# king159/Pair-Net

Hardware: AMD Instinct MI355X
Metric: images/sec (whole node), 100-query 800x1333, 1/2/4/8 MI355X (higher is better)
Workload: dtype f32

## Files before the change

include/pairnet_hip.h:

```cpp
#ifndef PAIRNET_HIP_H_
#define PAIRNET_HIP_H_

#include <stdint.h>

#ifdef __cplusplus
extern "C" {
#endif

#define PN_ABI_VERSION 34
int pn_abi_version(void);

#define PN_GEMM_RELU       1
#define PN_GEMM_A_COLMAJOR 2
#define PN_GEMM_FORCE_TILE 4
#define PN_GEMM_FORCE_SKINNY 8
#define PN_GEMM_FORCE_TILE64 16
#define PN_GEMM_FORCE_TILE128x64 32
#define PN_GEMM_RELU_AFTER_RES 128
#define PN_GEMM_GELU 256
#define PN_GEMM_RESERVE_SHIFT 16
#define PN_GEMM_RESERVE(n) ((((n) / 8) & 0x3ff) << PN_GEMM_RESERVE_SHIFT)
#define PN_GEMM_KSPLIT_SHIFT 26
#define PN_GEMM_KSPLIT(n) (((n) & 31) << PN_GEMM_KSPLIT_SHIFT)

// ... 408 lines not shown
int pn_layernorm_rows_bwd_f32(const float* dy, int64_t lddy, const float* x, int64_t ldx,
                              const float* gamma, float* dx, int64_t lddx, float* gxhat,
                              int64_t ldg, int64_t rows, int C, float eps, void* stream);
int pn_gelu_f32(const float* x, float* y, int64_t n, void* stream);
int pn_gelu_bwd_f32(const float* dy, const float* x, float* dx, int64_t n, void* stream);
int pn_window_attention_bwd_f32(const float* qkv, int64_t ldqkv, const float* qkv_bias,
                                const float* bias_table, const float* dout, int64_t lddo,
                                const float* out, int64_t ldo, float* dqkv, int64_t lddqkv,
                                float* dtable_part, int B, int H, int W, int C, int heads, int ws,
                                int shift, float scale, void* stream);
int pn_patch_merge_ln_bwd_f32(const float* dy, const float* x, const float* gamma, float* dx,
                              float* part, int nblocks, int B, int H, int W, int C, float eps,
                              int accumulate, void* stream);
int pn_conv_weight_bwd_layout_f32(const float* in, float* out, int Co, int T, int Ci, void* stream);
int pn_dropout_f32(const float* x, const float* res , float* y, int64_t n, float p,
                   uint64_t seed, uint32_t subseq, uint32_t step, uint32_t site, void* stream);
int pn_dropout_keep_u8(uint8_t* keep, int64_t n, float p, uint64_t seed, uint32_t subseq,
                       uint32_t step, uint32_t site, void* stream);

int pn_grad_norm_clip_f32(const float* g, int64_t n, float pre, float max_norm, float* out,
                          double* scratch, void* stream);
int pn_adamw_f32(float* p, const float* g, float* m, float* v, int64_t n, const int64_t* seg_off,
                 const float* seg_lr, const float* seg_wd, int nseg, float lr, double beta1,
                 double beta2, float eps, float weight_decay, int step, const float* clip, float pre,
                 void* stream);
int pn_adamw_guarded_f32(float* p, const float* g, float* m, float* v, int64_t n,
                         const int64_t* seg_off, const float* seg_lr, const float* seg_wd, int nseg,
                         float lr, double beta1, double beta2, float eps, float weight_decay,
                         int step, const float* clip, float pre, const int32_t* guard, void* stream);

int64_t pn_s3_bytes(int rows, int K);
int pn_s3_split_f32(const float* X, int64_t ld, const float* add, int add_rows, void* S, int rows,
                    int K, void* stream);
int pn_s3_join_f32(const void* S, float* X, int64_t ld, int rows, int K, void* stream);
typedef struct pn_gemm_s3_desc {
  const void* A;  const void* A2;  int32_t a2_from_col;
  const void* W;  const float* bias;
  int32_t M, N, K;
  int32_t relu;
  float* C;       int64_t ldc;
  void* CS;
  void* CS_pos;   const float* pos;  int32_t pos_rows;
  const void* res_s3;  const float* gamma;  const float* beta;  float eps;
  int32_t flags;
  int32_t act;  const float* res;  int64_t ldres;
} pn_gemm_s3_desc;
#define PN_GEMM_S3_TILE96 1
#define PN_GEMM_S3_TILE192 2
int pn_gemm_s3_f32(const pn_gemm_s3_desc* d, void* stream);
typedef struct pn_gemm_s3_ffn_desc {
  const void* X;  const void* W1;  const float* b1;
  const void* W2; const float* b2;
  int32_t M, N, K, F;
  int32_t act;
  float* C;       int64_t ldc;
  void* CS;
  void* CS_pos;   const float* pos;  int32_t pos_rows;
  const void* res_s3;  const float* gamma;  const float* beta;  float eps;
} pn_gemm_s3_ffn_desc;
int pn_gemm_s3_ffn_f32(const pn_gemm_s3_ffn_desc* d, void* stream);

int pn_uniform_f32(float* out, int64_t n, int nsites, uint32_t site_stride, uint64_t seed,
                   uint32_t rank, uint32_t step, uint32_t site, void* stream);
int pn_seg_targets(const int64_t* table, const int32_t* row_ind, const int32_t* col_ind,
                   const int32_t* lsa_status, int nlsa, const int64_t* gt_labels, int64_t gt_len,
                   int64_t out_len, int L, int B, int Q, int C, int64_t Mtot, int64_t* labels,
                   int64_t* matched, int32_t* mcount, int32_t* status, void* stream);
int pn_uncertain_points_f32(const float* maps, int64_t nmaps, const int64_t* matched, int64_t M,
                            int B, int Q, int h, int w, const float* cand, const float* tail, int S,
                            int k, int Np, uint32_t* keys, float* pts, void* stream);
int pn_point_sample_rows_f32(const void* maps, int maps_are_u8, int64_t nmaps, const int64_t* idx,
                             const float* pts, float* out, int64_t M, int h, int w, int Np,
                             void* stream);
int pn_mask_point_loss_f32(const float* x, const float* t, const int64_t* matched, int64_t M, int Np,
                           int L, int Ml, float w_mask, float w_dice, float dice_eps,
                           float num_total_masks, float* sums, float* out , float* coef,
                           void* stream);
int64_t pn_point_scatter_scratch_ints(int64_t M, int Np, int h, int w);
int pn_point_scatter_grad_f32(const float* coef, const float* pts, float* grad, int32_t* scratch,
                              int64_t M, int Np, int h, int w, void* stream);
int pn_ce_avg_f32(const float* logits, const int64_t* target, const float* class_weight, float* out,
                  int L, int rows, int C, float loss_weight, void* stream);
int pn_ce_avg_grad_f32(const float* logits, const int64_t* target, const float* class_weight,
                       float* grad, int L, int rows, int C, float loss_weight, void* stream);

int pn_rel_id_cost_f32(const float* rel, const float* sub, const float* obj, const int64_t* gt_rels,
                       int64_t rel_len, const int64_t* matched, int64_t Mtot, const int64_t* tab,
                       float* cost, int64_t cost_len, int B, int R, int Q, int C1, float w_s,
                       float w_o, float w_r, void* stream);
int pn_rel_targets(const int64_t* tab, const int32_t* row_ind, const int32_t* col_ind,
                   int64_t out_len, const int32_t* lsa_status, const int64_t* gt_rels,
                   int64_t rel_len, const int64_t* matched, int64_t Mtot, int B, int R, int Q, int C1,
                   int64_t* r_labels, int32_t* pos, int32_t* status, void* stream);
// ... 62 lines not shown
```

pair-net_amd/csrc/gemm_s3.hip:

```cpp
#include "common.h"
#include "s3_common.h"

__device__ __forceinline__ void s3_glds16(const void* g, void* l) {
  __builtin_amdgcn_global_load_lds((const __attribute__((address_space(1))) void*)g,
                                   (__attribute__((address_space(3))) void*)l, 16, 0, 0);
}

__device__ __forceinline__ int64_t pos8_offset(int row, int col, int N) {
  return ((((int64_t)(row >> 5) * (N >> 4) + (col >> 4)) * 2 + ((col >> 3) & 1)) * 32 + (row & 31)) * 8;
}

__global__ __launch_bounds__(256) void k_s3_split(const float* __restrict__ X, int64_t ld,
                                                  const float* __restrict__ add, int add_rows,
                                                  uint4* __restrict__ S, int R, int K) {
  const int KB = K >> 4;
  const int lane = threadIdx.x & 63;
  const int64_t piece = (int64_t)blockIdx.x * 4 + (threadIdx.x >> 6);
  const int64_t npieces = (int64_t)((R + 31) >> 5) * KB;
  if (piece >= npieces) return;
  const int rb = (int)(piece / KB), kb = (int)(piece - (int64_t)rb * KB);
  const int r = rb * 32 + (lane & 31), k = kb * 16 + (lane >> 5) * 8;
  float v[8];
  if (r < R) {
    const float4 a = ld4(X + (int64_t)r * ld + k), b = ld4(X + (int64_t)r * ld + k + 4);
    v[0] = a.x; v[1] = a.y; v[2] = a.z; v[3] = a.w; v[4] = b.x; v[5] = b.y; v[6] = b.z; v[7] = b.w;
    if (add) {
      const float* p = add + (int64_t)(r % add_rows) * K + k;
      const float4 c = ld4(p), d = ld4(p + 4);
      v[0] += c.x; v[1] += c.y; v[2] += c.z; v[3] += c.w; v[4] += d.x; v[5] += d.y; v[6] += d.z; v[7] += d.w;
    }
  } else {
#pragma unroll
    for (int i = 0; i < 8; ++i) v[i] = 0.f;
  }
  s3_frag p0, p1, p2;
  s3_split8(v, p0, p1, p2);
  uint4* o = S + piece * 192 + lane;
  o[0] = p0.u; o[64] = p1.u; o[128] = p2.u;
}

__global__ __launch_bounds__(256) void k_s3_join(const uint4* __restrict__ S, float* __restrict__ X,
                                                 int64_t ld, int R, int K) {
  const int KB = K >> 4;
  const int lane = threadIdx.x & 63;
  const int64_t piece = (int64_t)blockIdx.x * 4 + (threadIdx.x >> 6);
  const int64_t npieces = (int64_t)((R + 31) >> 5) * KB;
  if (piece >= npieces) return;
  const int rb = (int)(piece / KB), kb = (int)(piece - (int64_t)rb * KB);
  const int r = rb * 32 + (lane & 31), k = kb * 16 + (lane >> 5) * 8;
  if (r >= R) return;
  const uint4* in = S + piece * 192 + lane;
  s3_frag p0, p1, p2;
  p0.u = in[0]; p1.u = in[64]; p2.u = in[128];
  float v[8];
  s3_join8(p0, p1, p2, v);
  st4(X + (int64_t)r * ld + k, make_float4(v[0], v[1], v[2], v[3]));
  st4(X + (int64_t)r * ld + k + 4, make_float4(v[4], v[5], v[6], v[7]));
}

struct s3_args {
  const uint4* A; const uint4* A2; int a2_from_tile;
  const uint4* W; const float* bias;
  float* C; int64_t ldc; uint4* CS; uint4* CSP;
  const uint4* RES; const float* gamma; const float* beta; const float* pos; int pos_rows; float eps;
  int M, N, K, relu;
  const float* res; int64_t ldres;
  int nout;
};

__device__ __forceinline__ void s3_block_epilogue(const f32x16& acc, const s3_args& p, int rb, int n0,
// ... 648 lines not shown
        read(u & 1, as);
        if (u < 7) issueW1(c, u + 1);
        else issueW2(c, 0);
        if (u + 2 < 8) issueA(u + 2, as2, 1);
        __builtin_amdgcn_s_setprio(0);
        bar();
        mma(acc1);
        drain_bar();
        as = as == 2 ? 0 : as + 1;
      }
      make_pieces(c);
      bar();
#pragma unroll 1
      for (int s = 0; s < 8; ++s) {
        const int as2 = as == 0 ? 2 : as - 1;
        const bool more = c + 1 < NC;
        __builtin_amdgcn_s_setprio(1);
        read(s & 1, as);
        if (s < 7) issueW2(c, s + 1);
        else if (more) issueW1(c + 1, 0);
        if (s >= 6 && more) issueA(s - 6, as2, 1);
        __builtin_amdgcn_s_setprio(0);
        bar();
        mma(acc2);
        if (wave == s + 2) write_pieces(as2);
        if (more || s < 7) drain_bar();
        as = as == 2 ? 0 : as + 1;
      }
    }
  }
  s3_ln_epilogue(acc2, p, smem, rb0, wave * 32, wave, lane);
}

__global__ __launch_bounds__(256) void k_gemm_s3_narrow(const s3_args p, const int col0) {
  const int lane = threadIdx.x & 63;
  const int KB = p.K >> 4, RB = (p.M + 31) >> 5, ncb = (p.N - col0) >> 5;
  const int unit = blockIdx.x * 4 + (threadIdx.x >> 6);
  if (unit >= RB * ncb) return;
  const int rb = unit / ncb, cb = (col0 >> 5) + unit - rb * ncb;
  const uint4* ga = ((p.A2 && (cb >> 3) >= p.a2_from_tile) ? p.A2 : p.A) + (int64_t)rb * KB * 192 + lane;
  const uint4* gw = p.W + (int64_t)cb * KB * 192 + lane;
  f32x16 acc;
#pragma unroll
  for (int r = 0; r < 16; ++r) acc[r] = 0.f;
  constexpr int PA[6] = {2, 1, 0, 1, 0, 0}, PB[6] = {0, 1, 2, 0, 1, 0};
  constexpr int D = 4;
  s3_frag a[D][3], b[D][3];
  auto load = [&](int kb, int slot) {
#pragma unroll
    for (int q = 0; q < 3; ++q) { a[slot][q].u = ga[kb * 192 + q * 64]; b[slot][q].u = gw[kb * 192 + q * 64]; }
  };
#pragma unroll
  for (int d = 0; d < D; ++d)
    if (d < KB) load(d, d);
  for (int kb = 0; kb < KB; kb += D) {
#pragma unroll
    for (int d = 0; d < D; ++d) {
      if (kb + d >= KB) break;
#pragma unroll
      for (int q = 0; q < 6; ++q)
        acc = __builtin_amdgcn_mfma_f32_32x32x16_bf16(b[d][PB[q]].v, a[d][PA[q]].v, acc, 0, 0, 0);
      if (kb + d + D < KB) load(kb + d + D, d);
    }
  }
  s3_block_epilogue(acc, p, rb, cb * 32, lane);
}

extern "C" int64_t pn_s3_bytes(int rows, int K) {
  return (int64_t)((rows + 31) / 32) * (K / 16) * 3072;
}

extern "C" int pn_s3_split_f32(const float* X, int64_t ld, const float* add, int add_rows, void* S,
                               int rows, int K, void* stream) {
  if (!X || !S || rows <= 0 || K <= 0 || K % 16 || ld % 4 || (add && add_rows <= 0)) return PN_BAD_ARG;
  const int64_t np = (int64_t)((rows + 31) / 32) * (K / 16);
  k_s3_split<<<dim3((unsigned)((np + 3) / 4)), dim3(256), 0, (hipStream_t)stream>>>(
      X, ld, add, add ? add_rows : 1, (uint4*)S, rows, K);
  return PN_LAUNCH_CHECK();
}

extern "C" int pn_s3_join_f32(const void* S, float* X, int64_t ld, int rows, int K, void* stream) {
  if (!X || !S || rows <= 0 || K <= 0 || K % 16 || ld % 4) return PN_BAD_ARG;
  const int64_t np = (int64_t)((rows + 31) / 32) * (K / 16);
  k_s3_join<<<dim3((unsigned)((np + 3) / 4)), dim3(256), 0, (hipStream_t)stream>>>(
      (const uint4*)S, X, ld, rows, K);
  return PN_LAUNCH_CHECK();
}

extern "C" int pn_gemm_s3_ffn_f32(const pn_gemm_s3_ffn_desc* d, void* stream) {
  if (!d || !d->X || !d->W1 || !d->W2 || d->M <= 0) return PN_BAD_ARG;
  if (d->K != 256 || d->N != 256 || d->F <= 0 || d->F % 256) return PN_BAD_ARG;
  if (d->act != 1) return PN_BAD_ARG;
  if (!d->gamma || !d->beta) return PN_BAD_ARG;
  if (!d->C && !d->CS && !d->CS_pos) return PN_BAD_ARG;
  if (d->C && (d->ldc % 4 || d->ldc < d->N)) return PN_BAD_ARG;
  if (d->CS_pos && (!d->pos || d->pos_rows <= 0)) return PN_BAD_ARG;
  s3_args a;
  a.A = (const uint4*)d->X; a.A2 = nullptr; a.a2_from_tile = 0;
  a.W = (const uint4*)d->W2; a.bias = d->b2;
  a.C = d->C; a.ldc = d->ldc; a.CS = (uint4*)d->CS; a.CSP = (uint4*)d->CS_pos;
  a.RES = (const uint4*)d->res_s3; a.gamma = d->gamma; a.beta = d->beta; a.pos = d->pos;
  a.pos_rows = d->pos_rows; a.eps = d->eps;
  a.M = d->M; a.N = d->N; a.K = d->F; a.relu = 0; a.nout = d->N;
  a.res = nullptr; a.ldres = 0;
  const int RB = (d->M + 31) / 32, mt = (RB + 2) / 3;
  k_gemm_s3_ffn<<<dim3(mt), dim3(512), 0, (hipStream_t)stream>>>(a, (const uint4*)d->W1, d->b1);
  return PN_LAUNCH_CHECK();
}

extern "C" int pn_gemm_s3_f32(const pn_gemm_s3_desc* d, void* stream) {
  if (!d || !d->A || !d->W || d->M <= 0 || d->N <= 0 || d->K <= 0) return PN_BAD_ARG;
  if (d->K % 32 || d->N % 32) return PN_BAD_ARG;
  if (!d->C && !d->CS && !d->CS_pos) return PN_BAD_ARG;
  if (d->C && (d->ldc % 4 || d->ldc < d->N)) return PN_BAD_ARG;
  if (d->A2 && (d->a2_from_col <= 0 || d->a2_from_col % 256)) return PN_BAD_ARG;
  if (d->CS_pos && (!d->pos || d->pos_rows <= 0)) return PN_BAD_ARG;
  const bool ln = d->gamma != nullptr;
  if (ln && (d->N != 256 || !d->beta || d->relu)) return PN_BAD_ARG;
  if (!ln && d->res_s3) return PN_BAD_ARG;
  if (d->res && (ln || d->ldres % 4 || d->ldres < d->N)) return PN_BAD_ARG;
  if (d->act < 0 || d->act > 3 || (ln && d->act)) return PN_BAD_ARG;
  s3_args a;
  a.A = (const uint4*)d->A; a.A2 = (const uint4*)d->A2; a.a2_from_tile = d->A2 ? d->a2_from_col / 256 : 0;
  a.W = (const uint4*)d->W; a.bias = d->bias;
  a.C = d->C; a.ldc = d->ldc; a.CS = (uint4*)d->CS; a.CSP = (uint4*)d->CS_pos;
  a.RES = (const uint4*)d->res_s3; a.gamma = d->gamma; a.beta = d->beta; a.pos = d->pos;
  a.pos_rows = d->pos_rows; a.eps = d->eps;
  a.M = d->M; a.N = d->N; a.K = d->K; a.relu = d->act ? d->act : d->relu; a.nout = d->N;
  a.res = d->res; a.ldres = d->ldres;
  const int rem = d->N % 256;
  const bool narrow = !ln && !d->CS_pos && d->N > 256 && rem > 0 && rem <= 64;
  const int RB = (d->M + 31) / 32, mt = (RB + 2) / 3;
  bool wide = !ln && !d->CS_pos && (d->N - (narrow ? rem : 0)) >= 512 && !(d->flags & PN_GEMM_S3_TILE96);
  if (wide && !(d->flags & PN_GEMM_S3_TILE192)) {
    static int cus = 0;
    if (!cus) {
      int dev = 0;
      if (hipGetDevice(&dev) != hipSuccess ||
          hipDeviceGetAttribute(&cus, hipDeviceAttributeMultiprocessorCount, dev) != hipSuccess || cus <= 0)
// ... 29 lines not shown
```

pair-net_amd/head.py:

```python
import math
from collections import OrderedDict

import torch

from . import hip
from . import plans
from .plans import Arena, PlanCache, measure_bytes
from .config import ConfigDict

INSTANCE_OFFSET = 1000


def _decoder_param_shapes(prefix, num_layers, ffn_dim, out):
    for i in range(num_layers):
        p = "%s.layers.%d." % (prefix, i)
        for a in (0, 1):
            out[p + "attentions.%d.attn.in_proj_weight" % a] = (768, 256)
            out[p + "attentions.%d.attn.in_proj_bias" % a] = (768,)
            out[p + "attentions.%d.attn.out_proj.weight" % a] = (256, 256)
            out[p + "attentions.%d.attn.out_proj.bias" % a] = (256,)
        out[p + "ffns.0.layers.0.0.weight"] = (ffn_dim, 256)
        out[p + "ffns.0.layers.0.0.bias"] = (ffn_dim,)
        out[p + "ffns.0.layers.1.weight"] = (256, ffn_dim)
        out[p + "ffns.0.layers.1.bias"] = (256,)
# ... 70 lines not shown
        self.num_enc_layers = pixel_decoder.encoder.num_layers
        self.enc_ffn = pixel_decoder.encoder.transformerlayers.ffn_cfgs.feedforward_channels
        self.gn_groups = pixel_decoder.norm_cfg.num_groups
        self.num_dec_layers = transformer_decoder.num_layers
        self.dec_ffn = transformer_decoder.transformerlayers.ffn_cfgs.feedforward_channels
        self.num_rel_layers = relation_decoder.num_layers
        self.rel_ffn = relation_decoder.transformerlayers.ffn_cfgs.feedforward_channels
        self.rel_ffn_drop = float(relation_decoder.transformerlayers.ffn_cfgs.get("ffn_drop", 0.0))
        self.other_drop_rates = _drop_rates(dict(pixel_decoder=pixel_decoder,
                                                 transformer_decoder=transformer_decoder,
                                                 relation_decoder=relation_decoder))
        self.other_drop_rates.pop("relation_decoder.transformerlayers.ffn_cfgs.ffn_drop", None)
        self.test_cfg, self.train_cfg = test_cfg, train_cfg
        assert len(self.in_channels) == 4 and num_transformer_feat_level == 3
        assert num_obj_query <= 256 and num_rel_query <= 128
        self._params = OrderedDict(
            (k, torch.zeros(s)) for k, s in self.param_shapes().items())
        self.device = None
        self.w = None
        self._plans = PlanCache()
        self._arenas, self._post_arenas, self._consts, self._pe = {}, {}, {}, OrderedDict()
        self._dummies = {}
        self._post = OrderedDict()
        self._pan_jobs = []
        self.graph_after = 1
        self.exact_mask_order = True
        self.conv_algo = "winograd4"
        self.use_graphs = False
        self.grid_reserve = 0
        self.fuse_ppn_front = True
        self.fuse_mask_pack = True
        self.gather_mask_stencil = True
        self.fuse_encoder_ffn = 1
        self.fuse_lateral_upadd = False
        self.enc_fused_ln = ("proj", "ffn")
        self.group_input_convs = False
        self.gemm_arithmetic = "bf16x3"
        self.msda_s3_out = False
        self.fused_pair_masks = True
        self.init_weights()

    def param_shapes(self):
        s = OrderedDict()
        Q, R = self.num_obj_query, self.num_rel_query
        _decoder_param_shapes("relation_decoder", self.num_rel_layers, self.rel_ffn, s)
        s["rel_query_embed.weight"] = (R, 256)
        s["rel_query_embed2.weight"] = (2 * R, 256)
        s["rel_query_embed3.weight"] = (2 * R, 256)
        s["rel_query_feat.weight"] = (R, 256)
        for i, (ci, co) in enumerate(((1, 64), (64, 64), (64, 1))):
            s["update_importance.conv_layers.%d.0.weight" % i] = (co, ci, 7, 7)
            s["update_importance.conv_layers.%d.0.bias" % i] = (co,)
        pd = "pixel_decoder."
        for i in range(3):
            cin = self.in_channels[3 - i]
            s[pd + "input_convs.%d.conv.weight" % i] = (256, cin, 1, 1)
            s[pd + "input_convs.%d.conv.bias" % i] = (256,)
            s[pd + "input_convs.%d.gn.weight" % i] = (256,)
            s[pd + "input_convs.%d.gn.bias" % i] = (256,)
        for i in range(self.num_enc_layers):
            p = pd + "encoder.layers.%d." % i
            for name, n in (("sampling_offsets", 192), ("attention_weights", 96),
                            ("value_proj", 256), ("output_proj", 256)):
                s[p + "attentions.0.%s.weight" % name] = (n, 256)
                s[p + "attentions.0.%s.bias" % name] = (n,)
            s[p + "ffns.0.layers.0.0.weight"] = (self.enc_ffn, 256)
# ... 464 lines not shown
        for i in range(self.num_enc_layers):
            p = pd + "encoder.layers.%d." % i
            a = p + "attentions.0."
            hip.gemm(X2, w[a + "voa.weight"], pl.VOA, M=B * SN, N=544, K=256, lda=256, ldw=256,
                     ldc=544, bias=w[a + "voa.bias"], aadd=pl.enc_pos, ldaadd=256, aadd_rows=SN,
                     aadd_from_col=256)
            hip.msda(pl.VOA, 544, pl.VOA.view(-1)[256:], 544, pl.S, B, pl.shapes)
            if "proj" in self.enc_fused_ln:
                hip.linear_res_ln(pl.S.view(-1, 256), w[a + "output_proj.weight"],
                                  w[a + "output_proj.bias"], X2, w[p + "norms.0.weight"],
                                  w[p + "norms.0.bias"], X12)
            else:
                hip.linear(pl.S.view(-1, 256), w[a + "output_proj.weight"],
                           w[a + "output_proj.bias"], Y2, res=X2)
                hip.layernorm(Y2, w[p + "norms.0.weight"], w[p + "norms.0.bias"], X12)
            hip.linear(X12, w[p + "ffns.0.layers.0.0.weight"], w[p + "ffns.0.layers.0.0.bias"],
                       pl.H, relu=True)
            if "ffn" in self.enc_fused_ln:
                hip.linear_res_ln(pl.H, w[p + "ffns.0.layers.1.weight"],
                                  w[p + "ffns.0.layers.1.bias"], X12, w[p + "norms.1.weight"],
                                  w[p + "norms.1.bias"], X2)
            else:
                hip.linear(pl.H, w[p + "ffns.0.layers.1.weight"], w[p + "ffns.0.layers.1.bias"],
                           Y2, res=X12)
                hip.layernorm(Y2, w[p + "norms.1.weight"], w[p + "norms.1.bias"], X2)

    def _encoder_s3(self, pl):
        w, B, SN = self.w, pl.B, pl.SN
        pd = "pixel_decoder."
        M, F = B * SN, self.enc_ffn
        X2 = pl.X.view(-1, 256)
        pos8 = (pl.enc_pos8, SN)
        fuse_ffn = bool(getattr(self, "fuse_encoder_ffn", 0)) and F % 256 == 0
        hip.s3_split(X2, pl.XS)
        hip.s3_split(X2, pl.XPS, add=pl.enc_pos)
        for i in range(self.num_enc_layers):
            p = pd + "encoder.layers.%d." % i
            a = p + "attentions.0."
            last = i + 1 == self.num_enc_layers
            hip.gemm_s3(pl.XS, w[a + "voa.weight.s3"], M, 544, 256, bias=w[a + "voa.bias"],
                        out=pl.VOA.view(-1, 544), a2=pl.XPS, a2_from_col=256)
            if self.msda_s3_out:
                hip.msda(pl.VOA, 544, pl.VOA.view(-1)[256:], 544, pl.SS, B, pl.shapes, s3_out=True)
            else:
                hip.msda(pl.VOA, 544, pl.VOA.view(-1)[256:], 544, pl.S, B, pl.shapes)
                hip.s3_split(pl.S.view(-1, 256), pl.SS)
            hip.gemm_s3(pl.SS, w[a + "output_proj.weight.s3"], M, 256, 256,
                        bias=w[a + "output_proj.bias"], out_s3=pl.X1S, res_s3=pl.XS,
                        gamma=w[p + "norms.0.weight"], beta=w[p + "norms.0.bias"])
            tail = dict(res_s3=pl.X1S, gamma=w[p + "norms.1.weight"], beta=w[p + "norms.1.bias"],
                        out=X2 if last else None, out_s3=None if last else pl.XS,
                        out_s3_pos=None if last else pl.XPS, pos=pos8)
            if fuse_ffn:
                hip.gemm_s3_ffn(pl.X1S, w[p + "ffns.0.layers.0.0.weight.s3"],
                                w[p + "ffns.0.layers.1.weight.s3"], M, 256, 256, F,
                                b1=w[p + "ffns.0.layers.0.0.bias"],
                                b2=w[p + "ffns.0.layers.1.bias"], **tail)
                continue
            hip.gemm_s3(pl.X1S, w[p + "ffns.0.layers.0.0.weight.s3"], M, F, 256,
                        bias=w[p + "ffns.0.layers.0.0.bias"], relu=True, out_s3=pl.HS)
            hip.gemm_s3(pl.HS, w[p + "ffns.0.layers.1.weight.s3"], M, 256, F,
                        bias=w[p + "ffns.0.layers.1.bias"], **tail)

    def _mlp3(self, prefix, src, dst, pl):
        w = self.w
        hip.linear(src, w[prefix + ".0.weight"], w[prefix + ".0.bias"], pl.m1, relu=True)
        hip.linear(pl.m1, w[prefix + ".2.weight"], w[prefix + ".2.bias"], pl.m2, relu=True)
        hip.linear(pl.m2, w[prefix + ".4.weight"], w[prefix + ".4.bias"], dst)

    def _mask_logits(self, me, pl, out):
        Q = self.num_obj_query
        hip.gemm(me, pl.MF, out, M=Q, N=pl.HW2, K=256, lda=256, ldw=256, ldc=pl.HW2,
                 batch=pl.B, sA=Q * 256, sW=pl.HW2 * 256, sC=Q * pl.HW2)

    def _head_embed(self, q, pl, with_cls, full_mask, cls_out=None, mp_out=None, normed=False):
        w, B, Q = self.w, pl.B, self.num_obj_query
        cls_out = pl.cls if cls_out is None else cls_out
        mp_out = pl.MP if mp_out is None else mp_out
        if not normed:
            hip.layernorm(q, w["transformer_decoder.post_norm.weight"],
                          w["transformer_decoder.post_norm.bias"], pl.qn)
        if with_cls:
# ... 185 lines not shown
        hip.gather_rows(pl.MP, pl.obj_pos, pl.obj_seg, B, Q, R, pl.HW2)

    def _outputs(self, pl):
        B, Q, R = pl.B, self.num_obj_query, self.num_rel_query
        H2, W2 = pl.hw2
        return (dict(sub=pl.sub_cls, obj=pl.obj_cls, cls=pl.cls, rel=pl.rel, importance=pl.imp),
                dict(mask=pl.MP.view(B, Q, H2, W2), sub_seg=pl.sub_seg.view(B, R, H2, W2),
                     obj_seg=pl.obj_seg.view(B, R, H2, W2)))

    def _check_feats(self, feats, img_metas):
        pv = getattr(self, "_packed_version", None)
        if self.w is not None and pv is not None and pv != self._weights_version():
            self._drop_weight_state()
        B = len(img_metas)
        assert len(feats) == 4 and all(f.shape[0] == B for f in feats)
        nchw = all(f.is_contiguous() for f in feats)
        nhwc = not nchw and all(f.is_contiguous(memory_format=torch.channels_last) for f in feats)
        for f, c in zip(feats, self.in_channels):
            if not f.is_cuda or f.dtype != torch.float32 or f.shape[1] != c or not (nchw or nhwc):
                raise RuntimeError("feats must be fp32 [B,C,H,W] device tensors with channels %s, "
                                   "all contiguous or all in channels_last memory format"
                                   % self.in_channels)
        if self.device is None:
            self.to(feats[0].device)
        shapes = [tuple(feats[3 - l].shape[-2:]) for l in range(3)]
        self._feats_nhwc = nhwc
        return B, shapes, tuple(feats[0].shape[-2:])

    def _run_stage(self, which, pl, feats=None):
        cfg = (self.exact_mask_order, self.conv_algo, self.fuse_ppn_front, self.grid_reserve,
               tuple(self.enc_fused_ln), self.group_input_convs,
               getattr(self, "fuse_mask_pack", True), self.gemm_arithmetic, self.msda_s3_out,
               self._fused_pair_masks(), bool(getattr(self, "fuse_encoder_ffn", 0)),
               getattr(self, "gather_mask_stencil", True), getattr(self, "fuse_lateral_upadd", False))
        if pl.graph_cfg != cfg:
            pl.graph_a = pl.graph_b = None
            pl.graphs_a = OrderedDict()
            pl.graph_c = PlanCache(self.POST_VIEWS)
            pl.graph_cfg = cfg
        cur = torch.cuda.current_stream(self.device)
        pl.streams[cur.cuda_stream] = cur
        try:
            self._run_stage_on(which, pl, feats, cur)
        finally:
            plans.note_use(cur)

    def _run_stage_on(self, which, pl, feats, cur):
        if which == "a":
            if not pl.pe_waited:
                if pl.pe_ready.query():
                    pl.pe_waited = True
                else:
                    cur.wait_event(pl.pe_ready)
            ptrs = tuple(f.data_ptr() for f in feats)
            ent = pl.graphs_a.get(ptrs)
            if ent is None:
                if len(pl.graphs_a) >= self.STAGE_A_GRAPHS:
                    for k, e in pl.graphs_a.items():
                        if e["graph"] is None:
                            del pl.graphs_a[k]
                            break
                    else:
                        if plans.quiet(cur):
                            torch.cuda.current_stream(self.device).synchronize()
                            pl.graphs_a.popitem(last=False)
                if len(pl.graphs_a) < self.STAGE_A_GRAPHS:
# ... 331 lines not shown
```

pair-net_amd/hip.py:

```python
import contextlib
import ctypes as C
import os
import threading

import torch

from .build import LIB_PATH

LIB_PATH = os.environ.get("PAIRNET_LIB") or LIB_PATH

_i32, _i64, _f32, _vp = C.c_int32, C.c_int64, C.c_float, C.c_void_p

GEMM_RELU, GEMM_A_COLMAJOR, GEMM_FORCE_TILE, GEMM_FORCE_SKINNY = 1, 2, 4, 8
GEMM_GELU = 256
GEMM_FORCE_TILE64, GEMM_FORCE_TILE128x64 = 16, 32
GEMM_RELU_AFTER_RES = 128
GEMM_GROUP_MAX = 18


class GemmDesc(C.Structure):
    _fields_ = [("A", _vp), ("lda", _i64), ("strideA", _i64),
                ("Aadd", _vp), ("ldaadd", _i64), ("aadd_rows", _i32),
                ("aadd_from_col", _i32),
                ("W", _vp), ("ldw", _i64), ("strideW", _i64),
                ("bias", _vp),
                ("Res", _vp), ("ldres", _i64), ("strideRes", _i64),
                ("C", _vp), ("ldc", _i64), ("strideC", _i64),
                ("M", _i32), ("N", _i32), ("K", _i32), ("batch", _i32),
                ("flags", _i32),
                ("splitk_scratch", _vp), ("splitk_scratch_floats", _i64)]


class GemmS3Desc(C.Structure):
    _fields_ = [("A", _vp), ("A2", _vp), ("a2_from_col", _i32),
                ("W", _vp), ("bias", _vp),
                ("M", _i32), ("N", _i32), ("K", _i32), ("relu", _i32),
                ("C", _vp), ("ldc", _i64),
                ("CS", _vp),
                ("CS_pos", _vp), ("pos", _vp), ("pos_rows", _i32),
                ("res_s3", _vp), ("gamma", _vp), ("beta", _vp), ("eps", _f32), ("flags", _i32),
                ("act", _i32), ("res", _vp), ("ldres", _i64)]


class GemmS3FfnDesc(C.Structure):
    _fields_ = [("X", _vp), ("W1", _vp), ("b1", _vp), ("W2", _vp), ("b2", _vp),
                ("M", _i32), ("N", _i32), ("K", _i32), ("F", _i32), ("act", _i32),
                ("C", _vp), ("ldc", _i64),
                ("CS", _vp),
                ("CS_pos", _vp), ("pos", _vp), ("pos_rows", _i32),
                ("res_s3", _vp), ("gamma", _vp), ("beta", _vp), ("eps", _f32)]


_SIGS = {
    "pn_abi_version": (C.c_int, []),
    "pn_s3_bytes": (_i64, [_i32, _i32]),
    "pn_s3_split_f32": (C.c_int, [_vp, _i64, _vp, _i32, _vp, _i32, _i32, _vp]),
    "pn_s3_join_f32": (C.c_int, [_vp, _vp, _i64, _i32, _i32, _vp]),
    "pn_gemm_s3_f32": (C.c_int, [C.POINTER(GemmS3Desc), _vp]),
    "pn_gemm_s3_ffn_f32": (C.c_int, [C.POINTER(GemmS3FfnDesc), _vp]),
    "pn_gemm_f32": (C.c_int, [C.POINTER(GemmDesc), _vp]),
    "pn_gemm_variant": (C.c_int, [C.POINTER(GemmDesc)]),
    "pn_gemm_grid_size": (C.c_int, [C.POINTER(GemmDesc)]),
    "pn_gemm_wgs_per_cu": (C.c_int, []),
    "pn_gemm_group_f32": (C.c_int, [C.POINTER(GemmDesc), C.c_int, _vp]),
    "pn_conv2d_nhwc_f32": (C.c_int, [_vp, _vp, _vp, _vp] + [_i32] * 10 + [_vp]),
    "pn_conv2d_nhwc_ex_f32": (C.c_int, [_vp] * 5 + [_i32] * 10 + [_vp, _i64, _vp]),
    "pn_bottleneck_proj_f32": (C.c_int, [_vp] * 8 + [_i32] * 8 + [_vp, _i64, _vp]),
    "pn_stem7x7s2_f32": (C.c_int, [_vp, _vp, _vp, _vp, _i32, _i32, _i32, _i32, _vp]),
    "pn_maxpool3x3s2_nhwc_f32": (C.c_int, [_vp, _vp, _i32, _i32, _i32, _i32, _vp]),
    "pn_winograd_f23_input_f32": (C.c_int, [_vp, _vp, _i32, _i32, _i32, _i32, _vp]),
    "pn_winograd_f23_output_f32": (C.c_int, [_vp, _vp, _vp, _i32, _i32, _i32, _i32, _i32, _vp]),
    "pn_winograd_f43_input_f32": (C.c_int, [_vp, _vp, _i32, _i32, _i32, _i32, _vp]),
    "pn_winograd_f43_output_f32": (C.c_int, [_vp, _vp, _vp, _i32, _i32, _i32, _i32, _i32, _vp]),
    "pn_layernorm_f32": (C.c_int, [_vp, _vp, _vp, _vp, _i64, _i32, _f32, _vp]),
    "pn_layernorm_rows_s3_f32": (C.c_int, [_vp, _i64, _vp, _vp, _vp, _i64, _i32, _f32, _vp]),
    "pn_layernorm_rows_f32": (C.c_int, [_vp, _i64, _vp, _vp, _vp, _i64, _i64, _i32, _f32, _vp]),
    "pn_patch_merge_ln_f32": (C.c_int, [_vp, _vp, _vp, _vp, _i32, _i32, _i32, _i32, _f32, _vp]),
    "pn_patch_im2col4_f32": (C.c_int, [_vp, _vp, _i32, _i32, _i32, _vp]),
    "pn_window_attention_f32": (C.c_int, [_vp, _i64, _vp, _vp, _vp, _i64] + [_i32] * 7 +
                                [_f32, _vp]),
    "pn_window_attention_s3_f32": (C.c_int, [_vp, _i64, _vp, _vp, _vp] + [_i32] * 7 + [_f32, _vp]),
    "pn_groupnorm_nblk": (C.c_int, [_i64]),
    "pn_groupnorm_nhwc_f32": (C.c_int, [_vp, _vp, _vp, _vp, _vp, _i32, _i64, _i32,
                                        _i32, _f32, _i32, _i64, _i64, _vp]),
    "pn_groupnorm_upadd_nhwc_f32": (C.c_int, [_vp] * 6 + [_i32] * 7 + [_f32, _i64, _i64, _i64, _vp]),
    "pn_l2normalize_f32": (C.c_int, [_vp, _vp, _i64, _i32, _f32, _vp]),
    "pn_ffn_scratch_floats": (_i64, [_i32, _i32]),
    "pn_ffn_ln_f32": (C.c_int, [_vp] * 9 + [_i32, _i32, _i32, _f32, _vp]),
    "pn_ffn_ln2_f32": (C.c_int, [_vp] * 12 + [_i32, _i32, _i32, _f32, _vp]),
    "pn_msda_f32": (C.c_int, [_vp, _i64, _vp, _i64, _vp, _i32, _i32, C.POINTER(_i32),
                              C.POINTER(_i32), _vp]),
    "pn_msda_ex_f32": (C.c_int, [_vp, _i64, _vp, _i64, _vp, _i32, _i32, C.POINTER(_i32),
# ... 519 lines not shown
def layernorm(x, gamma, beta, out, eps=1e-5):
    rows = x.numel() // 256
    _check(lib().pn_layernorm_f32(_ptr(x), _ptr(gamma), _ptr(beta), _ptr(out), rows, 256,
                                  eps, _stream()), "pn_layernorm_f32")


def linear_res_ln(x, weight, bias, res, gamma, beta, out, eps=1e-5):
    M, ldx = _rowmajor(x)
    N, ldw = _rowmajor(weight)
    Mr, ldr = _rowmajor(res)
    Mo, ldo = _rowmajor(out)
    K = x.shape[1]
    assert Mr == M and Mo == M and N == 256 and weight.shape[1] == K
    nbytes = 4.0 * (M * K + N * K + 2 * M * N)
    _check(_launch("k_gemm_rowln", 2.0 * M * N * K, nbytes,
                   lambda: lib().pn_linear_res_ln_f32(_ptr(x), ldx, _ptr(weight), ldw, _ptr(bias),
                                                      _ptr(res), ldr, _ptr(gamma), _ptr(beta),
                                                      _ptr(out), ldo, M, N, K, eps, _stream()),
                   meta=(M, N, K, 1, False)), "pn_linear_res_ln_f32")


def s3_floats(rows, K):
    return ((rows + 31) // 32) * (K // 16) * 768


def pos8(pos):
    rows, cols = pos.shape
    rb = (rows + 31) // 32
    p = pos.new_zeros(rb * 32, cols)
    p[:rows] = pos
    return p.view(rb, 32, cols // 16, 2, 8).permute(0, 2, 3, 1, 4).contiguous()


def s3_split(x, out, add=None):
    rows, ld = _rowmajor(x)
    K = x.shape[1]
    assert out.numel() * out.element_size() >= s3_floats(rows, K) * 4
    ar = 0
    if add is not None:
        ar, lda = _rowmajor(add)
        assert lda == K and add.shape[1] == K
    _check(_launch("k_s3_split", 0.0, 10.0 * rows * K,
                   lambda: lib().pn_s3_split_f32(_ptr(x), ld, _ptr(add), ar, _ptr(out), rows, K,
                                                 _stream())), "pn_s3_split_f32")


def s3_join(s3, out):
    rows, ld = _rowmajor(out)
    _check(_launch("k_s3_join", 0.0, 10.0 * rows * out.shape[1],
                   lambda: lib().pn_s3_join_f32(_ptr(s3), _ptr(out), ld, rows, out.shape[1],
                                                _stream())), "pn_s3_join_f32")


def gemm_s3(a, w, M, N, K, *, bias=None, relu=False, out=None, out_s3=None, out_s3_pos=None,
            pos=None, a2=None, a2_from_col=0, res_s3=None, gamma=None, beta=None, eps=1e-5,
            tile96=False, tile192=False, gelu=False, res=None, relu_after=False):
    d = GemmS3Desc()
    d.A, d.A2, d.a2_from_col = _ptr(a), _ptr(a2), a2_from_col
    d.W, d.bias = _ptr(w), _ptr(bias)
    d.M, d.N, d.K, d.relu = M, N, K, int(relu)
    if out is not None:
        Mo, ldc = _rowmajor(out)
        assert Mo == M and out.shape[1] >= N
        d.C, d.ldc = _ptr(out), ldc
    d.CS, d.CS_pos = _ptr(out_s3), _ptr(out_s3_pos)
    if out_s3_pos is not None:
        pos, pr = pos
        assert pos.numel() == (pr + 31) // 32 * 32 * N
        d.pos, d.pos_rows = _ptr(pos), pr
    d.res_s3, d.gamma, d.beta, d.eps = _ptr(res_s3), _ptr(gamma), _ptr(beta), eps
    d.flags = (1 if tile96 else 0) | (2 if tile192 else 0)
    d.act = 3 if relu_after else 2 if gelu else 0
    if res is not None:
        Mr, ldr = _rowmajor(res)
        assert Mr == M and res.shape[1] >= N
        d.res, d.ldres = _ptr(res), ldr
    nbytes = 6.0 * (M * K + N * K) + (4.0 * M * N if out is not None else 0.0) + \
        6.0 * M * N * ((out_s3 is not None) + (out_s3_pos is not None) + (res_s3 is not None))
    name = "k_gemm_s3<ln>" if gamma is not None else "k_gemm_s3"
    _check(_launch(name, 2.0 * M * N * K, nbytes, lambda: lib().pn_gemm_s3_f32(C.byref(d), _stream()),
                   meta=(M, N, K, 1, False)), "pn_gemm_s3_f32")


def gemm_s3_ffn(x, w1, w2, M, N, K, F, *, b1=None, b2=None, res_s3=None, gamma=None, beta=None,
                eps=1e-5, out=None, out_s3=None, out_s3_pos=None, pos=None, gelu=False):
    d = GemmS3FfnDesc()
    d.X, d.W1, d.b1, d.W2, d.b2 = _ptr(x), _ptr(w1), _ptr(b1), _ptr(w2), _ptr(b2)
    d.M, d.N, d.K, d.F, d.act = M, N, K, F, 2 if gelu else 1
    if out is not None:
        Mo, ldc = _rowmajor(out)
        assert Mo == M and out.shape[1] >= N
        d.C, d.ldc = _ptr(out), ldc
    d.CS, d.CS_pos = _ptr(out_s3), _ptr(out_s3_pos)
    if out_s3_pos is not None:
        pos, pr = pos
        assert pos.numel() == (pr + 31) // 32 * 32 * N
        d.pos, d.pos_rows = _ptr(pos), pr
    d.res_s3, d.gamma, d.beta, d.eps = _ptr(res_s3), _ptr(gamma), _ptr(beta), eps
    nbytes = 6.0 * (M * K + 2 * F * K) + (4.0 * M * N if out is not None else 0.0) + \
        6.0 * M * N * ((out_s3 is not None) + (out_s3_pos is not None) + (res_s3 is not None))
    _check(_launch("k_gemm_s3_ffn", 2.0 * M * F * (K + N), nbytes,
                   lambda: lib().pn_gemm_s3_ffn_f32(C.byref(d), _stream()),
                   meta=(M, N, F, 1, False)), "pn_gemm_s3_ffn_f32")


def layernorm_rows(x, gamma, beta, out, eps=1e-5):
    rows, ldx = _rowmajor(x)
    ro, ldo = _rowmajor(out)
    assert ro == rows and out.shape[1] == x.shape[1]
    _check(_launch("k_ln_rows", 0.0, 8.0 * rows * x.shape[1],
                   lambda: lib().pn_layernorm_rows_f32(_ptr(x), ldx, _ptr(gamma), _ptr(beta),
                                                       _ptr(out), ldo, rows, x.shape[1], eps,
                                                       _stream())), "pn_layernorm_rows_f32")


def layernorm_rows_s3(x, gamma, beta, out_s3, eps=1e-5):
    rows, ldx = _rowmajor(x)
    Cc = x.shape[1]
    assert out_s3.numel() >= s3_floats(rows, Cc)
    _check(_launch("k_ln_rows<s3>", 0.0, 10.0 * rows * Cc,
                   lambda: lib().pn_layernorm_rows_s3_f32(_ptr(x), ldx, _ptr(gamma), _ptr(beta),
                                                          _ptr(out_s3), rows, Cc, eps, _stream())),
           "pn_layernorm_rows_s3_f32")


def patch_merge_ln(x, gamma, beta, out, B, H, W, C, eps=1e-5):
    _check(_launch("k_ln_rows<merge>", 0.0, 8.0 * B * H * W * C,
                   lambda: lib().pn_patch_merge_ln_f32(_ptr(x), _ptr(gamma), _ptr(beta), _ptr(out),
                                                       B, H, W, C, eps, _stream())),
           "pn_patch_merge_ln_f32")


def patch_im2col4(img, out, B, H, W):
    _check(_launch("k_patch_im2col", 0.0, 4.0 * B * H * W * 3 * 2.4,
                   lambda: lib().pn_patch_im2col4_f32(_ptr(img), _ptr(out), B, H, W, _stream())),
           "pn_patch_im2col4_f32")


# ... 1301 lines not shown
```

Measured before the change: 234.7.

## Fuse s3 split into encoder output-proj GEMM and merge dual splits

Adds a GEMM kernel that reads fp32 rows of the MSDA output directly and performs the three-way bf16 split in-kernel while loading A tiles. This removes the separate s3_split pass and its intermediate buffer round-trip in each encoder layer. It also merges the two initial splits (plain and with positional add) into one kernel that reads X once. The new kernel has its own hand-scheduled pipeline with a 3-stage A ring, and this could be slower than the pre-split path if the in-kernel conversion stalls the MFMA loop.

```diff
diff --git a/include/pairnet_hip.h b/include/pairnet_hip.h
--- a/include/pairnet_hip.h
+++ b/include/pairnet_hip.h
@@ -464,6 +464,8 @@
 int64_t pn_s3_bytes(int rows, int K);
 int pn_s3_split_f32(const float* X, int64_t ld, const float* add, int add_rows, void* S, int rows,
                     int K, void* stream);
+int pn_s3_split2_f32(const float* X, int64_t ld, const float* add, int add_rows, void* S, void* S_add,
+                     int rows, int K, void* stream);
 int pn_s3_join_f32(const void* S, float* X, int64_t ld, int rows, int K, void* stream);
 typedef struct pn_gemm_s3_desc {
   const void* A;  const void* A2;  int32_t a2_from_col;
@@ -491,6 +493,17 @@
   const void* res_s3;  const float* gamma;  const float* beta;  float eps;
 } pn_gemm_s3_ffn_desc;
 int pn_gemm_s3_ffn_f32(const pn_gemm_s3_ffn_desc* d, void* stream);
+typedef struct pn_gemm_s3_rows_desc {
+  const float* A;  int64_t lda;
+  const void* W;   const float* bias;
+  int32_t M, N, K;
+  int32_t act;
+  float* C;        int64_t ldc;
+  void* CS;
+  void* CS_pos;    const float* pos;  int32_t pos_rows;
+  const void* res_s3;  const float* gamma;  const float* beta;  float eps;
+} pn_gemm_s3_rows_desc;
+int pn_gemm_s3_rows_ln_f32(const pn_gemm_s3_rows_desc* d, void* stream);
 
 int pn_uniform_f32(float* out, int64_t n, int nsites, uint32_t site_stride, uint64_t seed,
                    uint32_t rank, uint32_t step, uint32_t site, void* stream);
diff --git a/pair-net_amd/csrc/gemm_s3.hip b/pair-net_amd/csrc/gemm_s3.hip
--- a/pair-net_amd/csrc/gemm_s3.hip
+++ b/pair-net_amd/csrc/gemm_s3.hip
@@ -36,6 +36,37 @@
   s3_frag p0, p1, p2;
   s3_split8(v, p0, p1, p2);
   uint4* o = S + piece * 192 + lane;
+  o[0] = p0.u; o[64] = p1.u; o[128] = p2.u;
+}
+
+__global__ __launch_bounds__(256) void k_s3_split2(const float* __restrict__ X, int64_t ld,
+                                                   const float* __restrict__ add, int add_rows,
+                                                   uint4* __restrict__ S, uint4* __restrict__ SP, int R, int K) {
+  const int KB = K >> 4;
+  const int lane = threadIdx.x & 63;
+  const int64_t piece = (int64_t)blockIdx.x * 4 + (threadIdx.x >> 6);
+  const int64_t npieces = (int64_t)((R + 31) >> 5) * KB;
+  if (piece >= npieces) return;
+  const int rb = (int)(piece / KB), kb = (int)(piece - (int64_t)rb * KB);
+  const int r = rb * 32 + (lane & 31), k = kb * 16 + (lane >> 5) * 8;
+  float v[8], w[8];
+  if (r < R) {
+    const float4 a = ld4(X + (int64_t)r * ld + k), b = ld4(X + (int64_t)r * ld + k + 4);
+    const float* p = add + (int64_t)(r % add_rows) * K + k;
+    const float4 c = ld4(p), d = ld4(p + 4);
+    v[0] = a.x; v[1] = a.y; v[2] = a.z; v[3] = a.w; v[4] = b.x; v[5] = b.y; v[6] = b.z; v[7] = b.w;
+    w[0] = a.x + c.x; w[1] = a.y + c.y; w[2] = a.z + c.z; w[3] = a.w + c.w;
+    w[4] = b.x + d.x; w[5] = b.y + d.y; w[6] = b.z + d.z; w[7] = b.w + d.w;
+  } else {
+#pragma unroll
+    for (int i = 0; i < 8; ++i) v[i] = w[i] = 0.f;
+  }
+  s3_frag p0, p1, p2;
+  s3_split8(v, p0, p1, p2);
+  uint4* o = S + piece * 192 + lane;
+  o[0] = p0.u; o[64] = p1.u; o[128] = p2.u;
+  s3_split8(w, p0, p1, p2);
+  o = SP + piece * 192 + lane;
   o[0] = p0.u; o[64] = p1.u; o[128] = p2.u;
 }
 
@@ -750,6 +781,140 @@
   s3_ln_epilogue(acc2, p, smem, rb0, wave * 32, wave, lane);
 }
 
+__global__ __launch_bounds__(512, 1) void k_gemm_s3_rows(const s3_args p, const float* __restrict__ Af,
+                                                         const int64_t lda) {
+  constexpr int MB = 3;
+  constexpr int AH = 9 * 64, AST = 2 * AH;
+  constexpr int BH = 24 * 64, BST = 2 * BH;
+  constexpr int BRING = 3 * AST;
+  __shared__ __attribute__((aligned(1024))) uint4 smem[3 * AST + 2 * BST];
+  const int tid = threadIdx.x, lane = tid & 63, wave = __builtin_amdgcn_readfirstlane(tid >> 6);
+  const int grp = wave >> 2, wq = wave & 3;
+  const int M = p.M, KB = p.K >> 4, S = KB >> 1;
+  const int RB = (M + 31) >> 5, mt = (RB + MB - 1) / MB;
+  const int rb0 = xcd_tile_index(blockIdx.x, mt) * MB;
+
+  const int cb = grp * 4 + wq;
+  const uint4* gW = p.W + (int64_t)cb * KB * 192;
+  const int lW = cb * 3 * 64;
+  const unsigned ul = lane;
+  auto issueB = [&](int s) {
+    const uint4* g = gW + (int64_t)s * 384;
+    const int base = BRING + (s & 1) * BST + lW;
+#pragma unroll
+    for (int h = 0; h < 2; ++h)
+#pragma unroll
+      for (int q = 0; q < 3; ++q) s3_glds16(g + (h * 192 + q * 64) + ul, &smem[base + h * BH + q * 64]);
+  };
+  const bool aw = wq < 3;
+  const int arow = (rb0 + wq) * 32 + (lane & 31);
+  const bool aok = aw && arow < M;
+  const float* ga = Af + (int64_t)(aok ? arow : 0) * lda + (lane >> 5) * 8;
+  auto loadA = [&](int s, int half, float4& x, float4& y) {
+    x = y = make_float4(0.f, 0.f, 0.f, 0.f);
+    if (aok) {
+      const float* g = ga + (2 * s + half) * 16;
+      x = ld4(g); y = ld4(g + 4);
+    }
+  };
+  auto writeA = [&](int as, int half, const float4& x, const float4& y) {
+    if (!aw) return;
+    const float v[8] = {x.x, x.y, x.z, x.w, y.x, y.y, y.z, y.w};
+    s3_frag q0, q1, q2;
+    s3_split8(v, q0, q1, q2);
+    uint4* d = smem + as * AST + half * AH + wq * 3 * 64 + lane;
+    d[0] = q0.u; d[64] = q1.u; d[128] = q2.u;
+  };
+  s3_frag a[2][MB][3], b[2][3];
+  f32x16 acc[MB];
+#pragma unroll
+  for (int m = 0; m < MB; ++m)
+#pragma unroll
+    for (int r = 0; r < 16; ++r) acc[m][r] = 0.f;
+  const int bfrag = cb * 3 * 64 + lane;
+  auto read = [&](int s, int as) {
+    const uint4* pa = smem + as * AST + lane;
+    const uint4* pb = smem + BRING + (s & 1) * BST + bfrag;
+#pragma unroll
+    for (int h = 0; h < 2; ++h) {
+#pragma unroll
+      for (int m = 0; m < MB; ++m)
+#pragma unroll
+        for (int q = 0; q < 3; ++q) a[h][m][q].u = pa[h * AH + (m * 3 + q) * 64];
+#pragma unroll
+      for (int q = 0; q < 3; ++q) b[h][q].u = pb[h * BH + q * 64];
+    }
+  };
+  auto mma = [&] {
+    constexpr int PA[6] = {2, 1, 0, 1, 0, 0}, PB[6] = {0, 1, 2, 0, 1, 0};
+#pragma unroll
+    for (int h = 0; h < 2; ++h)
+#pragma unroll
+      for (int q = 0; q < 6; ++q)
+#pragma unroll
+        for (int m = 0; m < MB; ++m)
+          acc[m] = __builtin_amdgcn_mfma_f32_32x32x16_bf16(b[h][PB[q]].v, a[h][m][PA[q]].v, acc[m], 0, 0, 0);
+    __builtin_amdgcn_sched_barrier(0);
+  };
+  auto bar = [&] {
+    __builtin_amdgcn_sched_barrier(0);
+    asm volatile("" ::: "memory");
+    __builtin_amdgcn_s_barrier();
+    asm volatile("" ::: "memory");
+    __builtin_amdgcn_sched_barrier(0);
+  };
+  auto drain_bar = [&] {
+    __builtin_amdgcn_sched_barrier(0);
+    __builtin_amdgcn_s_waitcnt(0x0070);
+    bar();
+  };
+  issueB(0);
+  {
+    float4 x0, y0, x1, y1;
+    loadA(0, grp, x0, y0);
+    if (grp == 1 && S > 1) loadA(1, 1, x1, y1);
+    writeA(0, grp, x0, y0);
+    if (grp == 1 && S > 1) writeA(1, 1, x1, y1);
+  }
+  drain_bar();
+  if (grp == 0) {
+    int as = 0;
+    for (int s = 0; s < S; ++s) {
+      const int as1 = as == 2 ? 0 : as + 1;
+      const bool more = s + 1 < S;
+      float4 hx, hy;
+      __builtin_amdgcn_s_setprio(1);
+      read(s, as);
+      if (more) { loadA(s + 1, 0, hx, hy); issueB(s + 1); }
+      __builtin_amdgcn_s_setprio(0);
+      bar();
+      mma();
+      if (more) writeA(as1, 0, hx, hy);
+      drain_bar();
+      as = as1;
+    }
+  } else {
+    bar();
+    int as = 0;
+    for (int s = 0; s < S; ++s) {
+      const int as2 = as == 0 ? 2 : as - 1;
+      const bool more2 = s + 2 < S;
+      float4 hx, hy;
+      __builtin_amdgcn_s_setprio(1);
+      read(s, as);
+      if (more2) loadA(s + 2, 1, hx, hy);
+      if (s + 1 < S) issueB(s + 1);
+      __builtin_amdgcn_s_setprio(0);
+      bar();
+      mma();
+      if (more2) writeA(as2, 1, hx, hy);
+      if (s + 1 < S) drain_bar();
+      as = as == 2 ? 0 : as + 1;
+    }
+  }
+  s3_ln_epilogue(acc, p, smem, rb0, wave * 32, wave, lane);
+}
+
 __global__ __launch_bounds__(256) void k_gemm_s3_narrow(const s3_args p, const int col0) {
   const int lane = threadIdx.x & 63;
   const int KB = p.K >> 4, RB = (p.M + 31) >> 5, ncb = (p.N - col0) >> 5;
@@ -794,6 +959,16 @@
   const int64_t np = (int64_t)((rows + 31) / 32) * (K / 16);
   k_s3_split<<<dim3((unsigned)((np + 3) / 4)), dim3(256), 0, (hipStream_t)stream>>>(
       X, ld, add, add ? add_rows : 1, (uint4*)S, rows, K);
+  return PN_LAUNCH_CHECK();
+}
+
+extern "C" int pn_s3_split2_f32(const float* X, int64_t ld, const float* add, int add_rows, void* S,
+                                void* S_add, int rows, int K, void* stream) {
+  if (!X || !S || !S_add || !add || add_rows <= 0 || rows <= 0 || K <= 0 || K % 16 || ld % 4)
+    return PN_BAD_ARG;
+  const int64_t np = (int64_t)((rows + 31) / 32) * (K / 16);
+  k_s3_split2<<<dim3((unsigned)((np + 3) / 4)), dim3(256), 0, (hipStream_t)stream>>>(
+      X, ld, add, add_rows, (uint4*)S, (uint4*)S_add, rows, K);
   return PN_LAUNCH_CHECK();
 }
 
@@ -823,6 +998,28 @@
   a.res = nullptr; a.ldres = 0;
   const int RB = (d->M + 31) / 32, mt = (RB + 2) / 3;
   k_gemm_s3_ffn<<<dim3(mt), dim3(512), 0, (hipStream_t)stream>>>(a, (const uint4*)d->W1, d->b1);
+  return PN_LAUNCH_CHECK();
+}
+
+extern "C" int pn_gemm_s3_rows_ln_f32(const pn_gemm_s3_rows_desc* d, void* stream) {
+  if (!d || !d->A || !d->W || d->M <= 0) return PN_BAD_ARG;
+  if (d->N != 256 || d->K <= 0 || d->K % 32) return PN_BAD_ARG;
+  if (d->lda % 4 || d->lda < d->K || ((uintptr_t)d->A & 15)) return PN_BAD_ARG;
+  if (d->act) return PN_BAD_ARG;
+  if (!d->gamma || !d->beta) return PN_BAD_ARG;
+  if (!d->C && !d->CS && !d->CS_pos) return PN_BAD_ARG;
+  if (d->C && (d->ldc % 4 || d->ldc < d->N)) return PN_BAD_ARG;
+  if (d->CS_pos && (!d->pos || d->pos_rows <= 0)) return PN_BAD_ARG;
+  s3_args a;
+  a.A = nullptr; a.A2 = nullptr; a.a2_from_tile = 0;
+  a.W = (const uint4*)d->W; a.bias = d->bias;
+  a.C = d->C; a.ldc = d->ldc; a.CS = (uint4*)d->CS; a.CSP = (uint4*)d->CS_pos;
+  a.RES = (const uint4*)d->res_s3; a.gamma = d->gamma; a.beta = d->beta; a.pos = d->pos;
+  a.pos_rows = d->pos_rows; a.eps = d->eps;
+  a.M = d->M; a.N = d->N; a.K = d->K; a.relu = 0; a.nout = d->N;
+  a.res = nullptr; a.ldres = 0;
+  const int RB = (d->M + 31) / 32, mt = (RB + 2) / 3;
+  k_gemm_s3_rows<<<dim3(mt), dim3(512), 0, (hipStream_t)stream>>>(a, d->A, d->lda);
   return PN_LAUNCH_CHECK();
 }
 
diff --git a/pair-net_amd/head.py b/pair-net_amd/head.py
--- a/pair-net_amd/head.py
+++ b/pair-net_amd/head.py
@@ -126,6 +126,7 @@
         self.fuse_mask_pack = True
         self.gather_mask_stencil = True
         self.fuse_encoder_ffn = 1
+        self.enc_proj_reads_rows = 1
         self.fuse_lateral_upadd = False
         self.enc_fused_ln = ("proj", "ffn")
         self.group_input_convs = False
@@ -656,8 +657,8 @@
         X2 = pl.X.view(-1, 256)
         pos8 = (pl.enc_pos8, SN)
         fuse_ffn = bool(getattr(self, "fuse_encoder_ffn", 0)) and F % 256 == 0
-        hip.s3_split(X2, pl.XS)
-        hip.s3_split(X2, pl.XPS, add=pl.enc_pos)
+        rows_proj = bool(getattr(self, "enc_proj_reads_rows", 0)) and not self.msda_s3_out
+        hip.s3_split(X2, pl.XS, add=pl.enc_pos, out_add=pl.XPS)
         for i in range(self.num_enc_layers):
             p = pd + "encoder.layers.%d." % i
             a = p + "attentions.0."
@@ -668,10 +669,15 @@
                 hip.msda(pl.VOA, 544, pl.VOA.view(-1)[256:], 544, pl.SS, B, pl.shapes, s3_out=True)
             else:
                 hip.msda(pl.VOA, 544, pl.VOA.view(-1)[256:], 544, pl.S, B, pl.shapes)
-                hip.s3_split(pl.S.view(-1, 256), pl.SS)
-            hip.gemm_s3(pl.SS, w[a + "output_proj.weight.s3"], M, 256, 256,
-                        bias=w[a + "output_proj.bias"], out_s3=pl.X1S, res_s3=pl.XS,
+                if not rows_proj:
+                    hip.s3_split(pl.S.view(-1, 256), pl.SS)
+            proj = dict(bias=w[a + "output_proj.bias"], out_s3=pl.X1S, res_s3=pl.XS,
                         gamma=w[p + "norms.0.weight"], beta=w[p + "norms.0.bias"])
+            if rows_proj:
+                hip.gemm_s3_rows_ln(pl.S.view(-1, 256), w[a + "output_proj.weight.s3"], M, 256, 256,
+                                    **proj)
+            else:
+                hip.gemm_s3(pl.SS, w[a + "output_proj.weight.s3"], M, 256, 256, **proj)
             tail = dict(res_s3=pl.X1S, gamma=w[p + "norms.1.weight"], beta=w[p + "norms.1.bias"],
                         out=X2 if last else None, out_s3=None if last else pl.XS,
                         out_s3_pos=None if last else pl.XPS, pos=pos8)
@@ -923,6 +929,7 @@
                tuple(self.enc_fused_ln), self.group_input_convs,
                getattr(self, "fuse_mask_pack", True), self.gemm_arithmetic, self.msda_s3_out,
                self._fused_pair_masks(), bool(getattr(self, "fuse_encoder_ffn", 0)),
+               bool(getattr(self, "enc_proj_reads_rows", 0)),
                getattr(self, "gather_mask_stencil", True), getattr(self, "fuse_lateral_upadd", False))
         if pl.graph_cfg != cfg:
             pl.graph_a = pl.graph_b = None
diff --git a/pair-net_amd/hip.py b/pair-net_amd/hip.py
--- a/pair-net_amd/hip.py
+++ b/pair-net_amd/hip.py
@@ -51,6 +51,16 @@
                 ("res_s3", _vp), ("gamma", _vp), ("beta", _vp), ("eps", _f32)]
 
 
+class GemmS3RowsDesc(C.Structure):
+    _fields_ = [("A", _vp), ("lda", _i64),
+                ("W", _vp), ("bias", _vp),
+                ("M", _i32), ("N", _i32), ("K", _i32), ("act", _i32),
+                ("C", _vp), ("ldc", _i64),
+                ("CS", _vp),
+                ("CS_pos", _vp), ("pos", _vp), ("pos_rows", _i32),
+                ("res_s3", _vp), ("gamma", _vp), ("beta", _vp), ("eps", _f32)]
+
+
 _SIGS = {
     "pn_abi_version": (C.c_int, []),
     "pn_s3_bytes": (_i64, [_i32, _i32]),
@@ -58,6 +68,8 @@
     "pn_s3_join_f32": (C.c_int, [_vp, _vp, _i64, _i32, _i32, _vp]),
     "pn_gemm_s3_f32": (C.c_int, [C.POINTER(GemmS3Desc), _vp]),
     "pn_gemm_s3_ffn_f32": (C.c_int, [C.POINTER(GemmS3FfnDesc), _vp]),
+    "pn_gemm_s3_rows_ln_f32": (C.c_int, [C.POINTER(GemmS3RowsDesc), _vp]),
+    "pn_s3_split2_f32": (C.c_int, [_vp, _i64, _vp, _i32, _vp, _vp, _i32, _i32, _vp]),
     "pn_gemm_f32": (C.c_int, [C.POINTER(GemmDesc), _vp]),
     "pn_gemm_variant": (C.c_int, [C.POINTER(GemmDesc)]),
     "pn_gemm_grid_size": (C.c_int, [C.POINTER(GemmDesc)]),
@@ -643,7 +655,7 @@
     return p.view(rb, 32, cols // 16, 2, 8).permute(0, 2, 3, 1, 4).contiguous()
 
 
-def s3_split(x, out, add=None):
+def s3_split(x, out, add=None, out_add=None):
     rows, ld = _rowmajor(x)
     K = x.shape[1]
     assert out.numel() * out.element_size() >= s3_floats(rows, K) * 4
@@ -651,6 +663,14 @@
     if add is not None:
         ar, lda = _rowmajor(add)
         assert lda == K and add.shape[1] == K
+    if out_add is not None:
+        assert add is not None
+        assert out_add.numel() * out_add.element_size() >= s3_floats(rows, K) * 4
+        _check(_launch("k_s3_split2", 0.0, 16.0 * rows * K,
+                       lambda: lib().pn_s3_split2_f32(_ptr(x), ld, _ptr(add), ar, _ptr(out),
+                                                      _ptr(out_add), rows, K, _stream())),
+               "pn_s3_split2_f32")
+        return
     _check(_launch("k_s3_split", 0.0, 10.0 * rows * K,
                    lambda: lib().pn_s3_split_f32(_ptr(x), ld, _ptr(add), ar, _ptr(out), rows, K,
                                                  _stream())), "pn_s3_split_f32")
@@ -715,6 +735,31 @@
                    meta=(M, N, F, 1, False)), "pn_gemm_s3_ffn_f32")
 
 
+def gemm_s3_rows_ln(a, w, M, N, K, *, bias=None, res_s3=None, gamma=None, beta=None, eps=1e-5,
+                    out=None, out_s3=None, out_s3_pos=None, pos=None):
+    d = GemmS3RowsDesc()
+    Ma, lda = _rowmajor(a)
+    assert Ma >= M
+    d.A, d.lda = _ptr(a), lda
+    d.W, d.bias = _ptr(w), _ptr(bias)
+    d.M, d.N, d.K, d.act = M, N, K, 0
+    if out is not None:
+        Mo, ldc = _rowmajor(out)
+        assert Mo == M and out.shape[1] >= N
+        d.C, d.ldc = _ptr(out), ldc
+    d.CS, d.CS_pos = _ptr(out_s3), _ptr(out_s3_pos)
+    if out_s3_pos is not None:
+        pos, pr = pos
+        assert pos.numel() == (pr + 31) // 32 * 32 * N
+        d.pos, d.pos_rows = _ptr(pos), pr
+    d.res_s3, d.gamma, d.beta, d.eps = _ptr(res_s3), _ptr(gamma), _ptr(beta), eps
+    nbytes = 4.0 * M * K + 6.0 * N * K + (4.0 * M * N if out is not None else 0.0) + \
+        6.0 * M * N * ((out_s3 is not None) + (out_s3_pos is not None) + (res_s3 is not None))
+    _check(_launch("k_gemm_s3_rows", 2.0 * M * N * K, nbytes,
+                   lambda: lib().pn_gemm_s3_rows_ln_f32(C.byref(d), _stream()),
+                   meta=(M, N, K, 1, False)), "pn_gemm_s3_rows_ln_f32")
+
+
 def layernorm_rows(x, gamma, beta, out, eps=1e-5):
     rows, ldx = _rowmajor(x)
     ro, ldo = _rowmajor(out)
```

New measurement: 237.3, median of 6. +1.1%, better.
